# antoine311200/sow

Measured on AMD Instinct MI355X. Metric: SoWLinear fwd+bwd tokens/s, llama_60m rank=50 (56-layer SoWLinear stack), higher is better.
Workload: dtype bf16

## Files before the change

### include/sow_amd.h

```cpp
#ifndef SOW_AMD_H
#define SOW_AMD_H

#include <stddef.h>
#include <stdint.h>

#ifdef __cplusplus
extern "C" {
#endif

#define SOW_DTYPE_F32 0
#define SOW_DTYPE_BF16 1
#define SOW_DTYPE_F16 2

#define SOW_PARAM_F32 0x100

#define SOW_OK 0
#define SOW_ERR_NULL (-1)
#define SOW_ERR_SHAPE (-2)
#define SOW_ERR_DTYPE (-3)
#define SOW_ERR_ALIGN (-4)
#define SOW_ERR_WORKSPACE (-5)
#define SOW_ERR_UNSUPPORTED (-6)

#define SOW_ACC_NONE 0
#define SOW_ACC_LOWRANK 1
#define SOW_ACC_DENSE 2

#define SOW_H_COLS 64

int sow_version(void);
const char* sow_error_string(int code);

int sow_set_switch(const char* name, int value);
int sow_get_switch(const char* name);

size_t sow_workspace_bytes(int64_t T, int d_in, int d_out, int r_live, int r_acc, int acc_kind, int dtype);
size_t sow_forward_workspace_bytes(int64_t T, int d_in, int d_out, int r_live, int r_acc, int acc_kind, int dtype);
size_t sow_h_save_elems(int64_t T, int r_live);

int sow_forward(const void* x, const void* A, const void* B, const void* acc_down, const void* acc_up, const void* bias,
                void* y, void* h_save, int64_t T, int d_in, int d_out, int r_live, int r_acc, int acc_kind, float scale,
                int dtype, void* workspace, size_t workspace_bytes, void* stream);

int sow_backward(const void* dy, const void* x, const void* h_save, const void* A, const void* B, const void* acc_down,
                 const void* acc_up, void* dx, void* dA, void* dB, void* dbias, int64_t T, int d_in, int d_out,
                 int r_live, int r_acc, int acc_kind, float scale, float grad_beta, int dtype, void* workspace,
                 size_t workspace_bytes, void* stream);

#define SOW_BWD_DATA 1
// ... 123 lines not shown
```

### sow_amd/_lib.py

```python
from __future__ import annotations

import ctypes
import os
from ctypes import POINTER, c_char_p, c_double, c_float, c_int, c_int64, c_size_t, c_void_p

_HERE = os.path.dirname(os.path.abspath(__file__))
LIB_PATH = os.environ.get("SOW_AMD_LIB") or os.path.join(_HERE, "lib", "libsow_amd.so")

F32, BF16, F16 = 0, 1, 2
PARAM_F32 = 0x100
ACC_NONE, ACC_LOWRANK, ACC_DENSE = 0, 1, 2
H_COLS = 64
BWD_DATA, BWD_WEIGHTS, BWD_WEIGHTS_PARTIAL, BWD_WEIGHTS_REDUCE = 1, 2, 4, 8
BWD_GROUP_SLABS = 16
ERR_SHAPE = -2
ERR_UNSUPPORTED = -6



class LayerArgs(ctypes.Structure):
    _fields_ = [("x", c_void_p), ("A", c_void_p), ("B", c_void_p), ("acc_down", c_void_p), ("acc_up", c_void_p),
                ("bias", c_void_p), ("y", c_void_p), ("h_save", c_void_p), ("dy", c_void_p), ("dx", c_void_p),
                ("dA", c_void_p), ("dB", c_void_p), ("dbias", c_void_p), ("T", c_int64), ("d_in", ctypes.c_int32),
                ("d_out", ctypes.c_int32), ("r_live", ctypes.c_int32), ("r_acc", ctypes.c_int32), ("acc_kind", ctypes.c_int32),
# ... 15 lines not shown
                ("in_dims", ctypes.c_int32 * TT_MAX_ORDER), ("out_dims", ctypes.c_int32 * TT_MAX_ORDER),
                ("rows", ctypes.c_int32), ("cols", ctypes.c_int32)]


class TtAdamItem(ctypes.Structure):
    _fields_ = [("m", TtDesc), ("v", TtDesc), ("param", c_void_p), ("grad", c_void_p), ("ld_param", c_int64),
                ("ld_grad", c_int64), ("step_size", c_float), ("lr_times_wd", c_float), ("has_state", ctypes.c_int32),
                ("workspace", c_void_p), ("workspace_bytes", c_size_t)]


SIGNATURES = {
    "sow_version": (c_int, []),
    "sow_error_string": (c_char_p, [c_int]),
    "sow_set_switch": (c_int, [c_char_p, c_int]),
    "sow_get_switch": (c_int, [c_char_p]),
    "sow_workspace_bytes": (c_size_t, [c_int64, c_int, c_int, c_int, c_int, c_int, c_int]),
    "sow_forward_workspace_bytes": (c_size_t, [c_int64, c_int, c_int, c_int, c_int, c_int, c_int]),
    "sow_h_save_elems": (c_size_t, [c_int64, c_int]),
    "sow_forward": (c_int, [c_void_p] * 8 + [c_int64, c_int, c_int, c_int, c_int, c_int, c_float, c_int, c_void_p,
                                               c_size_t, c_void_p]),
    "sow_backward": (c_int, [c_void_p] * 11 + [c_int64, c_int, c_int, c_int, c_int, c_int, c_float, c_float, c_int,
                                                 c_void_p, c_size_t, c_void_p]),
    "sow_backward_ex": (c_int, [c_void_p] * 11 + [c_int64, c_int, c_int, c_int, c_int, c_int, c_float, c_float, c_int,
                                    c_void_p, c_size_t, c_int, c_void_p]),
    "sow_forward_group": (c_int, [POINTER(LayerArgs), c_int, c_int, c_void_p]),
    "sow_backward_group": (c_int, [POINTER(LayerArgs), c_int, c_int, c_int, c_void_p]),
    "sow_forward_shared": (c_int, [POINTER(LayerArgs), c_int, c_int, c_void_p]),
    "sow_backward_shared": (c_int, [POINTER(LayerArgs), c_int, c_int, c_int, c_void_p]),
    "sow_backward_group_reduce_desc": (c_int, [POINTER(LayerArgs), c_int, c_int, c_int, c_void_p, POINTER(c_int)]),
    "sow_backward_group_plan": (c_int, [POINTER(LayerArgs), c_int, c_int, c_int, POINTER(c_int)]),
# ... 57 lines not shown
        msg = load().sow_error_string(code).decode()
        raise SowLibraryError(f"libsow_amd {what} failed with code {code}: {msg}")


class switch:

    def __init__(self, **values):
        self.values = values
        self.old = {}

    @staticmethod
    def _forget_sizes():
        from . import ops
        ops._WS_BYTES.clear()
        ops._FWD_WS_BYTES.clear()

    def __enter__(self):
        lib = load()
        for k, v in self.values.items():
            self.old[k] = lib.sow_get_switch(k.encode())
            check(lib.sow_set_switch(k.encode(), int(v)), f"sow_set_switch({k})")
        self._forget_sizes()
        return self

    def __exit__(self, *exc):
        lib = load()
        for k, v in self.old.items():
            lib.sow_set_switch(k.encode(), v)
        self._forget_sizes()
        return False
# ... 1 lines not shown
```

### sow_amd/csrc/api.hip

```cpp
#include "kernels.hpp"
#include <cstring>
#include <vector>
#include <cstdio>
#include <cstdlib>

namespace sow {

template <typename T, typename TO>
__global__ __launch_bounds__(256) void colsum_kernel(const T* M, int64_t ld, int64_t rows, int D, TO* out, float beta) {
  __shared__ float red[4][64];
  const int c = blockIdx.x * 64 + (threadIdx.x & 63), w = threadIdx.x >> 6;
  float s = 0.f;
  if (c < D)
    for (int64_t i = w; i < rows; i += 4) s += to_f32(M[i * ld + c]);
  red[w][threadIdx.x & 63] = s;
  __syncthreads();
  if (w == 0 && c < D) {
    float v = red[0][threadIdx.x] + red[1][threadIdx.x] + red[2][threadIdx.x] + red[3][threadIdx.x];
    if (beta != 0.f) v += beta * to_f32(out[c]);
    out[c] = from_f32<TO>(v);
  }
}
static int launch_colsum(const void* dy, int64_t T, int d_out, void* dbias, float beta, int dtype, int out_dtype,
                         hipStream_t stream) {
// ... 9 lines not shown
  else if (dtype == SOW_F16 && o32)
    hipLaunchKernelGGL((colsum_kernel<f16_t, float>), grid, dim3(256), 0, stream, (const f16_t*)dy, (int64_t)d_out, T, d_out, (float*)dbias, beta);
  else if (dtype == SOW_F16)
    hipLaunchKernelGGL((colsum_kernel<f16_t, f16_t>), grid, dim3(256), 0, stream, (const f16_t*)dy, (int64_t)d_out, T, d_out, (f16_t*)dbias, beta);
  else
    return SOW_ERR_DTYPE;
  SOW_CHECK_LAUNCH();
  return SOW_OK;
}
}

namespace sow {
static const char* const kSwitchNames[SW_COUNT] = {"FORCE_CHAIN_V1", "NO_SHORT_SPLIT", "NO_FUSED_H", "FORCE_GEMM_V1", "TN_NARROW",
                                                   "NO_GEMM3S",      "GEMM3S",         "GEMM3",      "NO_GROUPED",     "NO_PERSIST",     "NO_NT_STORE",    "NT_LOAD",        "NO_PAIR_FLUSH",  "F32_EXACT",
                                                   "NO_PARK16",      "TN_NO_NT_LOAD",  "NO_TN_ROWS",     "GEMM4",          "NO_GEMM4H",      "NO_CHAIN3F",     "NO_TN_F32Q",     "NO_SPLITK",
                                                   "NO_WIDE_CHAIN",  "NO_SHARED_X",    "NO_RAGGED",      "NO_RAGGED_GEMM"};
static std::atomic<int> g_switch[SW_COUNT];
static std::once_flag g_switch_once;
static void switches_from_env() {
  for (int i = 0; i < SW_COUNT; ++i) {
    char name[64];
    snprintf(name, sizeof name, "SOW_AMD_%s", kSwitchNames[i]);
    const char* v = getenv(name);
    const bool tri = i == SW_GEMM3S || i == SW_GEMM3 || i == SW_GEMM4;
    g_switch[i].store(!v ? -1 : (tri ? (v[0] != '0') : 1), std::memory_order_relaxed);
  }
}
int sw(int which) {
  std::call_once(g_switch_once, switches_from_env);
  return g_switch[which].load(std::memory_order_relaxed);
}
}

using namespace sow;

static inline size_t al256(size_t v) { return (v + 255) & ~(size_t)255; }
static inline size_t esize(int dtype) { return dtype == SOW_F32 ? 4 : 2; }
static inline bool ok_dtype(int d) { return d == SOW_F32 || d == SOW_BF16 || d == SOW_F16; }
static inline bool al4p(const void* p) { return (reinterpret_cast<uintptr_t>(p) & 3) == 0; }
static inline bool al16p(const void* p) { return (reinterpret_cast<uintptr_t>(p) & 15) == 0; }
static inline int split_dtype(int d, bool* pf) {
  *pf = (d & SOW_PARAM_F32) != 0;
  const int cd = d & ~SOW_PARAM_F32;
  if (!ok_dtype(cd) || (*pf && cd == SOW_F32)) return -1;
  return cd;
}
static inline bool flagged(int d) { return (d & SOW_PARAM_F32) != 0; }

constexpr int SHORT_NTB = 128;
// ... 46 lines not shown
    const int g4 = sw(SW_GEMM4);
    const int64_t work = (int64_t)ceil_div(M, 256) * ceil_div(N, 256) * gemm4_splits(M, N, K, false, ws, ws_bytes);
    if (!sw_on(SW_FORCE_GEMM_V1) && (g4 > 0 || (g4 < 0 && work >= 120)) &&
        gemm4_supported(A, lda, B, ldb, transB, nullptr, 0, nullptr, 0, C, ldc, bias, M, N, K, dtype))
      return launch_gemm4(A, lda, B, ldb, transB, nullptr, 0, nullptr, 0, 0, C, ldc, bias, M, N, K, alpha, beta, stream, ws,
                          ws_bytes, dtype);
    return launch_gemm(A, lda, false, B, ldb, transB, C, ldc, bias, M, N, K, alpha, beta, dtype, stream);
  }
  if (gemm2_supported(A, lda, B, ldb, transB, nullptr, 0, nullptr, 0, C, ldc, bias, M, N, K, dtype))
    return launch_gemm2(A, lda, B, ldb, transB, nullptr, 0, nullptr, 0, 0, C, ldc, bias, M, N, K, alpha, beta, stream, ws, ws_bytes);
  return launch_gemm(A, lda, false, B, ldb, transB, C, ldc, bias, M, N, K, alpha, beta, dtype, stream);
}

extern "C" {

int sow_version(void) { return 116; }

int sow_set_switch(const char* name, int value) {
  if (!name) return SOW_ERR_NULL;
  (void)sw(0);
  for (int i = 0; i < SW_COUNT; ++i)
    if (!strcmp(name, kSwitchNames[i])) {
      g_switch[i].store(value < 0 ? -1 : (value != 0), std::memory_order_relaxed);
      return SOW_OK;
    }
  return SOW_ERR_UNSUPPORTED;
}

#ifdef SOW_STAMPS
int sow_debug_set_stamps(void* buf) {
  g_chain2_stamps = buf;
  return SOW_OK;
}
#endif

int sow_get_switch(const char* name) {
  if (!name) return SOW_ERR_NULL;
  for (int i = 0; i < SW_COUNT; ++i)
// ... 254 lines not shown
    if (acc_kind == SOW_ACC_LOWRANK) {
      rc = wide_chain(x, y, acc_down, r_acc, acc_up, d_out, nullptr, nullptr, T, d_in, d_out, r_acc, 1.f, 1.f, 0.f, false, dtype,
                      ws, w, workspace_bytes, stream, true);
      if (rc) return rc;
      beta = 1.f;
    } else if (acc_kind == SOW_ACC_DENSE) {
      rc = rag_dense_product(x, d_in, acc_down, d_out, false, y, d_out, T, d_out, d_in, dtype, stream);
      if (rc) return rc;
      beta = 1.f;
    }
    return wide_chain(x, y, A, r_live, B, d_out, h_save, bias, T, d_in, d_out, r_live, 1.f, scale, beta, false, dtype, ws, w,
                      workspace_bytes, stream, true);
  }
  if (acc_kind == SOW_ACC_DENSE) {
    if (r_live <= 64 && h_save) {
      if (gemm4h_supported(x, d_in, acc_down, d_out, false, A, r_live, B, d_out, y, d_out, bias, h_save, T, d_out, d_in, r_live,
                           dtype))
        return launch_gemm4h(x, d_in, acc_down, d_out, false, A, r_live, B, d_out, y, d_out, bias, h_save, T, d_out, d_in,
                             r_live, scale, dtype, stream);
      if (gemm2h_supported(x, d_in, acc_down, d_out, false, A, r_live, B, d_out, y, d_out, bias, h_save, T, d_out, d_in,
                           r_live, dtype))
        return launch_gemm2h(x, d_in, acc_down, d_out, false, A, r_live, B, d_out, y, d_out, bias, h_save, T, d_out, d_in,
                             r_live, scale, stream);
      ChainParams ph{};
      ph.X = x, ph.Y = nullptr, ph.Hsave = h_save, ph.bias = nullptr;
      ph.M = T, ph.ldx = d_in, ph.ldy = d_out, ph.D1 = d_in, ph.D2 = 0;
      ph.F1b = A, ph.ldf1b = r_live, ph.F2b = B, ph.ldf2b = d_out, ph.rb = r_live;
      ph.scale = scale, ph.beta = 0.f;
      set_planes(ph, ws, w, workspace_bytes);
      if (chain2_supported(ph, dtype) &&
          gemm2_supported(x, d_in, acc_down, d_out, false, h_save, 64, B, d_out, y, d_out, bias, T, d_out, d_in, dtype)) {
        rc = SOW_ERR_UNSUPPORTED;
        if (ws && workspace_bytes >= w.total) rc = launch_chain_short(ph, dtype, false, (float*)(ws + w.off_hp), stream);
        if (rc == SOW_ERR_UNSUPPORTED) rc = launch_chain2(ph, false, dtype, stream);
// ... 131 lines not shown
    rc = wide_chain(dy, dx, B, d_out, A, r_live, dh, nullptr, T, d_out, d_in, r_live, scale, 1.f, beta, true, dtype, ws, w,
                    workspace_bytes, stream, true);
    if (rc) return rc;
    do_data = false;
  }
  if (!do_data) {
  } else if (acc_kind == SOW_ACC_DENSE) {
    if (r_live <= 64) {
      ChainParams pd{};
      pd.X = dy, pd.Y = nullptr, pd.Hsave = dh, pd.bias = nullptr;
      pd.M = T, pd.ldx = d_out, pd.ldy = d_in, pd.D1 = d_out, pd.D2 = 0;
      pd.F1b = B, pd.ldf1b = d_out, pd.F2b = A, pd.ldf2b = r_live, pd.rb = r_live;
      pd.scale = scale, pd.beta = 0.f;
      set_planes(pd, ws, w, workspace_bytes);
      void* apad = ws + w.off_apad;
      if (gemm4h_supported(dy, d_out, acc_down, d_out, true, B, d_out, A, r_live, dx, d_in, nullptr, dh, T, d_in, d_out, r_live,
                           dtype)) {
        rc = launch_gemm4h(dy, d_out, acc_down, d_out, true, B, d_out, A, r_live, dx, d_in, nullptr, dh, T, d_in, d_out, r_live,
                           scale, dtype, stream);
        if (rc) return rc;
        data_done = true;
      } else if (gemm2h_supported(dy, d_out, acc_down, d_out, true, B, d_out, A, r_live, dx, d_in, nullptr, dh, T, d_in, d_out,
                           r_live, dtype)) {
        rc = launch_gemm2h(dy, d_out, acc_down, d_out, true, B, d_out, A, r_live, dx, d_in, nullptr, dh, T, d_in, d_out,
                           r_live, scale, stream);
        if (rc) return rc;
        data_done = true;
      } else if (chain2_supported(pd, dtype) &&
          gemm2_supported(dy, d_out, acc_down, d_out, true, dh, 64, apad, 64, dx, d_in, nullptr, T, d_in, d_out, dtype)) {
        const bool pad_fused = (int64_t)ceil_div(T, 64) * 64 >= d_in;
        if (pad_fused) pd.pad_src = A, pd.pad_dst = apad, pd.pad_rows = d_in, pd.pad_r = r_live;
        rc = SOW_ERR_UNSUPPORTED;
        if (short_hp_bytes(T, d_in, d_out, r_live, dtype)) rc = launch_chain_short(pd, dtype, true, (float*)(ws + w.off_hp), stream);
        if (rc == SOW_ERR_UNSUPPORTED) rc = launch_chain2(pd, true, dtype, stream);
// ... 214 lines not shown
  ChainParams batch[C2_MAXG];
  Gemm2hArgs gbatch[4];
  int nb = 0, ng = 0, rc;
  for (int i = 0; i < n; ++i) {
    const sow_layer_args& L = layers[i];
    if ((rc = check_layer(L, false))) return rc;
    if (L.T == 0) continue;
    const WsPlan w{};
    if (group_chain_params(L, false, dtype, w, &batch[nb])) {
      if (++nb == C2_MAXG) {
        if ((rc = launch_chain2_group(batch, nb, false, dtype, stream))) return rc;
        nb = 0;
      }
      continue;
    }
    if (L.acc_kind == SOW_ACC_DENSE && L.r_live <= 64 && L.h_save &&
        gemm4h_supported(L.x, L.d_in, L.acc_down, L.d_out, false, L.A, L.r_live, L.B, L.d_out, L.y, L.d_out, L.bias, L.h_save, L.T,
                         L.d_out, L.d_in, L.r_live, dtype)) {
      if ((rc = launch_gemm4h(L.x, L.d_in, L.acc_down, L.d_out, false, L.A, L.r_live, L.B, L.d_out, L.y, L.d_out, L.bias, L.h_save,
                              L.T, L.d_out, L.d_in, L.r_live, L.scale, dtype, stream)))
        return rc;
      continue;
    }
    if (L.acc_kind == SOW_ACC_DENSE && L.r_live <= 64 && L.h_save && !sw_on(SW_NO_GROUPED) &&
        gemm2h_supported(L.x, L.d_in, L.acc_down, L.d_out, false, L.A, L.r_live, L.B, L.d_out, L.y, L.d_out, L.bias, L.h_save, L.T,
                         L.d_out, L.d_in, L.r_live, dtype)) {
      gbatch[ng] = Gemm2hArgs{L.x, L.acc_down, L.A, L.B, L.y, L.bias, L.h_save, L.T, L.d_in, L.d_out, L.r_live, L.d_out, L.d_out,
                              L.d_out, L.d_in, L.r_live, L.scale};
      if (++ng == 4) {
        if ((rc = launch_gemm2h_group(gbatch, ng, false, stream))) return rc;
        ng = 0;
      }
      continue;
    }
    rc = sow_forward(L.x, L.A, L.B, L.acc_down, L.acc_up, L.bias, L.y, L.h_save, L.T, L.d_in, L.d_out, L.r_live, L.r_acc,
                     L.acc_kind, L.scale, dtype, L.workspace, L.workspace_bytes, stream_);
    if (rc) return rc;
// ... 40 lines not shown
    for (int i = 0; i < n; ++i) {
      const sow_layer_args& L = layers[i];
      if (L.T == 0) {
        if ((rc = single(L, SOW_BWD_DATA | (phases & ~SOW_BWD_DATA)))) return rc;
        continue;
      }
      const WsPlan w = plan(L);
      if (L.workspace_bytes < w.total + 255) return SOW_ERR_WORKSPACE;
      void* dh = ws_base(L.workspace) + w.off_dh;
      if (group_chain_params(L, true, dtype, w, &batch[nb])) {
        if (++nb == C2_MAXG) {
          if ((rc = launch_chain2_group(batch, nb, true, dtype, stream))) return rc;
          nb = 0;
        }
      } else if (L.acc_kind == SOW_ACC_DENSE && L.r_live <= 64 &&
                 gemm4h_supported(L.dy, L.d_out, L.acc_down, L.d_out, true, L.B, L.d_out, L.A, L.r_live, L.dx, L.d_in, nullptr, dh,
                                  L.T, L.d_in, L.d_out, L.r_live, dtype)) {
        if ((rc = launch_gemm4h(L.dy, L.d_out, L.acc_down, L.d_out, true, L.B, L.d_out, L.A, L.r_live, L.dx, L.d_in, nullptr, dh,
                                L.T, L.d_in, L.d_out, L.r_live, L.scale, dtype, stream)))
          return rc;
      } else if (L.acc_kind == SOW_ACC_DENSE && L.r_live <= 64 && !sw_on(SW_NO_GROUPED) &&
                 gemm2h_supported(L.dy, L.d_out, L.acc_down, L.d_out, true, L.B, L.d_out, L.A, L.r_live, L.dx, L.d_in, nullptr, dh,
                                  L.T, L.d_in, L.d_out, L.r_live, dtype)) {
        gbatch[ng] = Gemm2hArgs{L.dy, L.acc_down, L.B, L.A, L.dx, nullptr, dh, L.T, L.d_out, L.d_out, L.d_out, L.r_live, L.d_in,
                                L.d_in, L.d_out, L.r_live, L.scale};
        if (++ng == 4) {
          if ((rc = launch_gemm2h_group(gbatch, ng, true, stream))) return rc;
          ng = 0;
        }
      } else if ((rc = single(L, SOW_BWD_DATA)))
        return rc;
    }
    if (ng && (rc = launch_gemm2h_group(gbatch, ng, true, stream))) return rc;
    if (nb && (rc = launch_chain2_group(batch, nb, true, dtype, stream))) return rc;
  }
// ... 351 lines not shown
```

### sow_amd/csrc/common.hpp

```cpp
#pragma once
#include <hip/hip_runtime.h>
#include <stdint.h>

#include <atomic>
#include <mutex>

#include "../../include/sow_amd.h"

namespace sow {

typedef __bf16 bf16_t;
typedef __attribute__((ext_vector_type(8))) __bf16 bf16x8;
typedef __attribute__((ext_vector_type(4))) __bf16 bf16x4;
typedef __attribute__((ext_vector_type(2))) __bf16 bf16x2;
typedef _Float16 f16_t;
typedef __attribute__((ext_vector_type(8))) _Float16 f16x8;
typedef __attribute__((ext_vector_type(2))) _Float16 f16x2;
typedef __attribute__((ext_vector_type(16))) float f32x16;
typedef __attribute__((ext_vector_type(4))) float f32x4;
typedef __attribute__((ext_vector_type(2))) float f32x2;
typedef __attribute__((ext_vector_type(4))) uint32_t u32x4;
typedef __attribute__((ext_vector_type(2))) uint32_t u32x2;

enum : int { SOW_F32 = 0, SOW_BF16 = 1, SOW_F16 = 2 };
// ... 110 lines not shown
  SW_NT_LOAD,
  SW_NO_PAIR_FLUSH,
  SW_F32_EXACT,
  SW_NO_PARK16,
  SW_TN_NO_NT_LOAD,
  SW_NO_TN_ROWS,
  SW_GEMM4,
  SW_NO_GEMM4H,
  SW_NO_CHAIN3F,
  SW_NO_TN_F32Q,
  SW_NO_SPLITK,
  SW_NO_WIDE_CHAIN,
  SW_NO_SHARED_X,
  SW_NO_RAGGED,
  SW_NO_RAGGED_GEMM,
  SW_COUNT
};
int sw(int which);
inline bool sw_on(int which) { return sw(which) > 0; }

#ifdef SOW_GEMM_NO_NT
#define SOW_GEMM_NT(M) false
#else
#define SOW_GEMM_NT(M) ((M) >= 8192)
#endif

#define SOW_CHECK_LAUNCH()                     \
  do {                                         \
    hipError_t e__ = hipGetLastError();        \
    if (e__ != hipSuccess) return (int)e__;    \
// ... 4 lines not shown
```

### sow_amd/csrc/kernels.hpp

```cpp
#pragma once
#include "common.hpp"

namespace sow {
struct ChainParams {
  const void* X;
  void* Y;
  const void *F1a, *F1b, *F2a, *F2b;
  void* Hsave;
  const void* bias;
  int64_t M, ldx, ldy, ldf1a, ldf1b, ldf2a, ldf2b;
  int D1, D2, ra, rb;
  float scale, beta;
  int fast_factors;
  const void* pad_src;
  void* pad_dst;
  int pad_rows, pad_r;
  int ntb, st_per, sl_per;
  float* Hpartial;
  const void* Hload;
  int nt_store;
  int nt_load;
  int pair_flush;
  void* planes;
  size_t planes_bytes;
// ... 151 lines not shown
                 float alpha, float beta, hipStream_t stream);
bool gemm4_supported(const void* A, int64_t lda, const void* B, int64_t ldb, bool nt, const void* A2, int64_t lda2,
                     const void* B2, int64_t ldb2, const void* C, int64_t ldc, const void* bias, int64_t M, int N, int K,
                     int dtype);
int launch_gemm4(const void* A, int64_t lda, const void* B, int64_t ldb, bool nt, const void* A2, int64_t lda2,
                 const void* B2, int64_t ldb2, int k2, void* C, int64_t ldc, const void* bias, int64_t M, int N, int K,
                 float alpha, float beta, hipStream_t stream, void* ws = nullptr, size_t ws_bytes = 0, int dtype = SOW_BF16);
size_t gemm4_splitk_bytes(int64_t M, int N, int K, bool has_ext);
int gemm4_splits(int64_t M, int N, int K, bool has_ext, const void* ws, size_t ws_bytes);
bool gemm4h_supported(const void* X, int64_t ldx, const void* W, int64_t ldw, bool nt, const void* F, int64_t ldf,
                      const void* G, int64_t ldg, const void* C, int64_t ldc, const void* bias, const void* H, int64_t M,
                      int N, int K, int r, int dtype);
int launch_gemm4h(const void* X, int64_t ldx, const void* W, int64_t ldw, bool nt, const void* F, int64_t ldf,
                  const void* G, int64_t ldg, void* C, int64_t ldc, const void* bias, void* H, int64_t M, int N, int K,
                  int r, float hscale, int dtype, hipStream_t stream);
bool gemm2h_supported(const void* X, int64_t ldx, const void* W, int64_t ldw, bool nt, const void* F, int64_t ldf,
                      const void* G, int64_t ldg, const void* C, int64_t ldc, const void* bias, const void* H, int64_t M,
                      int N, int K, int r, int dtype);
int launch_gemm2h(const void* X, int64_t ldx, const void* W, int64_t ldw, bool nt, const void* F, int64_t ldf,
                  const void* G, int64_t ldg, void* C, int64_t ldc, const void* bias, void* H, int64_t M, int N, int K,
                  int r, float hscale, hipStream_t stream);
struct Gemm2hArgs {
  const void *X, *W, *F, *G;
  void* C;
  const void* bias;
  void* H;
  int64_t M, ldx, ldw, ldf, ldg, ldc;
  int N, K, r;
  float hscale;
};
// ... 53 lines not shown
```

Before: 8.865 million.

## Add gemm5h fused dense plus low-rank GEMM with H output for wide-N backward

Adds a new bf16/f16 kernel for dense-accumulator layers. It fuses the dense GEMM with the low-rank H projection and its correction into one pass. It uses a 128x512 output tile, a three-stage LDS ring filled by direct-to-LDS DMA, and MFMA 16x16x32, with each dispatch path trying it before the existing gemm4h. By default it runs only for the backward data pass, N up to 512 and large token counts (at least 192 row panels). The aim is to read each X row panel once for the whole output width and to overlap loads with MFMA work. The cost is heavy LDS use per block, which may limit occupancy, and more complex edge patching for ragged F and G.

```diff
diff --git a/include/sow_amd.h b/include/sow_amd.h
--- a/include/sow_amd.h
+++ b/include/sow_amd.h
@@ -33,6 +33,8 @@
 
 int sow_set_switch(const char* name, int value);
 int sow_get_switch(const char* name);
+
+int sow_dense_h_kernel(int64_t T, int d_in, int d_out, int r_live, int dtype, int backward);
 
 size_t sow_workspace_bytes(int64_t T, int d_in, int d_out, int r_live, int r_acc, int acc_kind, int dtype);
 size_t sow_forward_workspace_bytes(int64_t T, int d_in, int d_out, int r_live, int r_acc, int acc_kind, int dtype);
diff --git a/sow_amd/_lib.py b/sow_amd/_lib.py
--- a/sow_amd/_lib.py
+++ b/sow_amd/_lib.py
@@ -53,6 +53,7 @@
     "sow_error_string": (c_char_p, [c_int]),
     "sow_set_switch": (c_int, [c_char_p, c_int]),
     "sow_get_switch": (c_int, [c_char_p]),
+    "sow_dense_h_kernel": (c_int, [c_int64, c_int, c_int, c_int, c_int, c_int]),
     "sow_workspace_bytes": (c_size_t, [c_int64, c_int, c_int, c_int, c_int, c_int, c_int]),
     "sow_forward_workspace_bytes": (c_size_t, [c_int64, c_int, c_int, c_int, c_int, c_int, c_int]),
     "sow_h_save_elems": (c_size_t, [c_int64, c_int]),
@@ -140,6 +141,7 @@
         from . import ops
         ops._WS_BYTES.clear()
         ops._FWD_WS_BYTES.clear()
+        ops._GEMM_WS_BYTES.clear()
 
     def __enter__(self):
         lib = load()
diff --git a/sow_amd/csrc/api.hip b/sow_amd/csrc/api.hip
--- a/sow_amd/csrc/api.hip
+++ b/sow_amd/csrc/api.hip
@@ -47,7 +47,7 @@
 static const char* const kSwitchNames[SW_COUNT] = {"FORCE_CHAIN_V1", "NO_SHORT_SPLIT", "NO_FUSED_H", "FORCE_GEMM_V1", "TN_NARROW",
                                                    "NO_GEMM3S",      "GEMM3S",         "GEMM3",      "NO_GROUPED",     "NO_PERSIST",     "NO_NT_STORE",    "NT_LOAD",        "NO_PAIR_FLUSH",  "F32_EXACT",
                                                    "NO_PARK16",      "TN_NO_NT_LOAD",  "NO_TN_ROWS",     "GEMM4",          "NO_GEMM4H",      "NO_CHAIN3F",     "NO_TN_F32Q",     "NO_SPLITK",
-                                                   "NO_WIDE_CHAIN",  "NO_SHARED_X",    "NO_RAGGED",      "NO_RAGGED_GEMM"};
+                                                   "NO_WIDE_CHAIN",  "NO_SHARED_X",    "NO_RAGGED",      "NO_RAGGED_GEMM", "GEMM5H"};
 static std::atomic<int> g_switch[SW_COUNT];
 static std::once_flag g_switch_once;
 static void switches_from_env() {
@@ -56,7 +56,10 @@
     snprintf(name, sizeof name, "SOW_AMD_%s", kSwitchNames[i]);
     const char* v = getenv(name);
     const bool tri = i == SW_GEMM3S || i == SW_GEMM3 || i == SW_GEMM4;
-    g_switch[i].store(!v ? -1 : (tri ? (v[0] != '0') : 1), std::memory_order_relaxed);
+    if (i == SW_GEMM5H)
+      g_switch[i].store(!v ? -1 : (v[0] >= '0' && v[0] <= '2' ? v[0] - '0' : 1), std::memory_order_relaxed);
+    else
+      g_switch[i].store(!v ? -1 : (tri ? (v[0] != '0') : 1), std::memory_order_relaxed);
   }
 }
 int sw(int which) {
@@ -66,6 +69,16 @@
 }
 
 using namespace sow;
+
+static int launch_dense_h(const void* X, int64_t ldx, const void* W, int64_t ldw, bool nt, const void* F, int64_t ldf,
+                          const void* G, int64_t ldg, void* C, int64_t ldc, const void* bias, void* H, int64_t M, int N, int K,
+                          int r, float hscale, int dtype, hipStream_t stream) {
+  if (gemm5h_supported(X, ldx, W, ldw, nt, F, ldf, G, ldg, C, ldc, bias, H, M, N, K, r, dtype))
+    return launch_gemm5h(X, ldx, W, ldw, nt, F, ldf, G, ldg, C, ldc, bias, H, M, N, K, r, hscale, dtype, stream);
+  if (gemm4h_supported(X, ldx, W, ldw, nt, F, ldf, G, ldg, C, ldc, bias, H, M, N, K, r, dtype))
+    return launch_gemm4h(X, ldx, W, ldw, nt, F, ldf, G, ldg, C, ldc, bias, H, M, N, K, r, hscale, dtype, stream);
+  return SOW_ERR_UNSUPPORTED;
+}
 
 static inline size_t al256(size_t v) { return (v + 255) & ~(size_t)255; }
 static inline size_t esize(int dtype) { return dtype == SOW_F32 ? 4 : 2; }
@@ -142,14 +155,24 @@
 
 extern "C" {
 
-int sow_version(void) { return 116; }
+int sow_version(void) { return 117; }
+
+int sow_dense_h_kernel(int64_t T, int d_in, int d_out, int r_live, int dtype, int backward) {
+  const void* a = reinterpret_cast<const void*>(uintptr_t(256));
+  const bool nt = backward != 0;
+  const int N = nt ? d_in : d_out, K = nt ? d_out : d_in;
+  const int64_t ldf = nt ? d_out : r_live, ldg = nt ? r_live : d_out;
+  if (gemm5h_supported(a, K, a, d_out, nt, a, ldf, a, ldg, a, N, nullptr, a, T, N, K, r_live, dtype)) return 5;
+  if (gemm4h_supported(a, K, a, d_out, nt, a, ldf, a, ldg, a, N, nullptr, a, T, N, K, r_live, dtype)) return 4;
+  return 0;
+}
 
 int sow_set_switch(const char* name, int value) {
   if (!name) return SOW_ERR_NULL;
   (void)sw(0);
   for (int i = 0; i < SW_COUNT; ++i)
     if (!strcmp(name, kSwitchNames[i])) {
-      g_switch[i].store(value < 0 ? -1 : (value != 0), std::memory_order_relaxed);
+      g_switch[i].store(value < 0 ? -1 : (i == SW_GEMM5H && value == 2 ? 2 : (value != 0)), std::memory_order_relaxed);
       return SOW_OK;
     }
   return SOW_ERR_UNSUPPORTED;
@@ -434,10 +457,9 @@
   }
   if (acc_kind == SOW_ACC_DENSE) {
     if (r_live <= 64 && h_save) {
-      if (gemm4h_supported(x, d_in, acc_down, d_out, false, A, r_live, B, d_out, y, d_out, bias, h_save, T, d_out, d_in, r_live,
-                           dtype))
-        return launch_gemm4h(x, d_in, acc_down, d_out, false, A, r_live, B, d_out, y, d_out, bias, h_save, T, d_out, d_in,
-                             r_live, scale, dtype, stream);
+      rc = launch_dense_h(x, d_in, acc_down, d_out, false, A, r_live, B, d_out, y, d_out, bias, h_save, T, d_out, d_in, r_live,
+                          scale, dtype, stream);
+      if (rc != SOW_ERR_UNSUPPORTED) return rc;
       if (gemm2h_supported(x, d_in, acc_down, d_out, false, A, r_live, B, d_out, y, d_out, bias, h_save, T, d_out, d_in,
                            r_live, dtype))
         return launch_gemm2h(x, d_in, acc_down, d_out, false, A, r_live, B, d_out, y, d_out, bias, h_save, T, d_out, d_in,
@@ -599,10 +621,9 @@
       pd.scale = scale, pd.beta = 0.f;
       set_planes(pd, ws, w, workspace_bytes);
       void* apad = ws + w.off_apad;
-      if (gemm4h_supported(dy, d_out, acc_down, d_out, true, B, d_out, A, r_live, dx, d_in, nullptr, dh, T, d_in, d_out, r_live,
-                           dtype)) {
-        rc = launch_gemm4h(dy, d_out, acc_down, d_out, true, B, d_out, A, r_live, dx, d_in, nullptr, dh, T, d_in, d_out, r_live,
-                           scale, dtype, stream);
+      rc = launch_dense_h(dy, d_out, acc_down, d_out, true, B, d_out, A, r_live, dx, d_in, nullptr, dh, T, d_in, d_out, r_live,
+                          scale, dtype, stream);
+      if (rc != SOW_ERR_UNSUPPORTED) {
         if (rc) return rc;
         data_done = true;
       } else if (gemm2h_supported(dy, d_out, acc_down, d_out, true, B, d_out, A, r_live, dx, d_in, nullptr, dh, T, d_in, d_out,
@@ -847,13 +868,13 @@
       }
       continue;
     }
-    if (L.acc_kind == SOW_ACC_DENSE && L.r_live <= 64 && L.h_save &&
-        gemm4h_supported(L.x, L.d_in, L.acc_down, L.d_out, false, L.A, L.r_live, L.B, L.d_out, L.y, L.d_out, L.bias, L.h_save, L.T,
-                         L.d_out, L.d_in, L.r_live, dtype)) {
-      if ((rc = launch_gemm4h(L.x, L.d_in, L.acc_down, L.d_out, false, L.A, L.r_live, L.B, L.d_out, L.y, L.d_out, L.bias, L.h_save,
-                              L.T, L.d_out, L.d_in, L.r_live, L.scale, dtype, stream)))
-        return rc;
-      continue;
+    if (L.acc_kind == SOW_ACC_DENSE && L.r_live <= 64 && L.h_save) {
+      rc = launch_dense_h(L.x, L.d_in, L.acc_down, L.d_out, false, L.A, L.r_live, L.B, L.d_out, L.y, L.d_out, L.bias, L.h_save, L.T,
+                          L.d_out, L.d_in, L.r_live, L.scale, dtype, stream);
+      if (rc != SOW_ERR_UNSUPPORTED) {
+        if (rc) return rc;
+        continue;
+      }
     }
     if (L.acc_kind == SOW_ACC_DENSE && L.r_live <= 64 && L.h_save && !sw_on(SW_NO_GROUPED) &&
         gemm2h_supported(L.x, L.d_in, L.acc_down, L.d_out, false, L.A, L.r_live, L.B, L.d_out, L.y, L.d_out, L.bias, L.h_save, L.T,
@@ -924,11 +945,9 @@
           nb = 0;
         }
       } else if (L.acc_kind == SOW_ACC_DENSE && L.r_live <= 64 &&
-                 gemm4h_supported(L.dy, L.d_out, L.acc_down, L.d_out, true, L.B, L.d_out, L.A, L.r_live, L.dx, L.d_in, nullptr, dh,
-                                  L.T, L.d_in, L.d_out, L.r_live, dtype)) {
-        if ((rc = launch_gemm4h(L.dy, L.d_out, L.acc_down, L.d_out, true, L.B, L.d_out, L.A, L.r_live, L.dx, L.d_in, nullptr, dh,
-                                L.T, L.d_in, L.d_out, L.r_live, L.scale, dtype, stream)))
-          return rc;
+                 (rc = launch_dense_h(L.dy, L.d_out, L.acc_down, L.d_out, true, L.B, L.d_out, L.A, L.r_live, L.dx, L.d_in, nullptr,
+                                      dh, L.T, L.d_in, L.d_out, L.r_live, L.scale, dtype, stream)) != SOW_ERR_UNSUPPORTED) {
+        if (rc) return rc;
       } else if (L.acc_kind == SOW_ACC_DENSE && L.r_live <= 64 && !sw_on(SW_NO_GROUPED) &&
                  gemm2h_supported(L.dy, L.d_out, L.acc_down, L.d_out, true, L.B, L.d_out, L.A, L.r_live, L.dx, L.d_in, nullptr, dh,
                                   L.T, L.d_in, L.d_out, L.r_live, dtype)) {
diff --git a/sow_amd/csrc/common.hpp b/sow_amd/csrc/common.hpp
--- a/sow_amd/csrc/common.hpp
+++ b/sow_amd/csrc/common.hpp
@@ -148,6 +148,7 @@
   SW_NO_SHARED_X,
   SW_NO_RAGGED,
   SW_NO_RAGGED_GEMM,
+  SW_GEMM5H,
   SW_COUNT
 };
 int sw(int which);
diff --git a/sow_amd/csrc/gemm5h.hip b/sow_amd/csrc/gemm5h.hip
--- /dev/null
+++ b/sow_amd/csrc/gemm5h.hip
@@ -0,0 +1,418 @@
+#include "kernels.hpp"
+#include "lds_dma.hpp"
+#include <type_traits>
+
+namespace sow {
+
+constexpr int G5_BM = 128, G5_BN = 512, G5_BK = 32;
+constexpr int G5_THREADS = 512;
+constexpr int G5_XOFF = 0, G5_WOFF = 8192, G5_FOFF = G5_WOFF + 32768;
+constexpr int G5_STAGE = G5_FOFF + 4096;
+constexpr int G5_RING = 3 * G5_STAGE;
+constexpr int G5_HIMG = G5_RING;
+constexpr int G5_LDS = G5_RING + 16384;
+constexpr int G5_SCR_LD = 132;
+constexpr int G5_SCR = 16 * G5_SCR_LD * 4;
+static_assert(8 * G5_SCR <= G5_RING, "the epilogue scratch lives in the ring");
+static_assert(G5_STAGE % 256 == 0, "the k-major fragment addresses XOR their low byte");
+
+struct Gemm5Params {
+  const bf16_t* X;
+  const bf16_t* W;
+  const bf16_t* F;
+  const bf16_t* G;
+  bf16_t* C;
+  const bf16_t* bias;
+  bf16_t* Hout;
+  int64_t M, ldx, ldw, ldf, ldg, ldc;
+  int N, K, r;
+  int k2e;
+  float hscale;
+  int nt_store;
+};
+
+template <typename T> __device__ __forceinline__ f32x4 g5_mfma(u32x4 a, u32x4 b, f32x4 c);
+template <> __device__ __forceinline__ f32x4 g5_mfma<bf16_t>(u32x4 a, u32x4 b, f32x4 c) {
+  return __builtin_amdgcn_mfma_f32_16x16x32_bf16(as_bf16x8(a), as_bf16x8(b), c, 0, 0, 0);
+}
+template <> __device__ __forceinline__ f32x4 g5_mfma<f16_t>(u32x4 a, u32x4 b, f32x4 c) {
+  return __builtin_amdgcn_mfma_f32_16x16x32_f16(as_v8<f16_t>(a), as_v8<f16_t>(b), c, 0, 0, 0);
+}
+
+template <int OFF> __device__ __forceinline__ void g5_rd128(u32x4& d, uint32_t a) {
+  asm volatile("ds_read_b128 %0, %1 offset:%2" : "=v"(d) : "v"(a), "n"(OFF) : "memory");
+}
+template <int OFF> __device__ __forceinline__ void g5_rdtr(u32x2& d, uint32_t a) {
+  asm volatile("ds_read_b64_tr_b16 %0, %1 offset:%2" : "=v"(d) : "v"(a), "n"(OFF) : "memory");
+}
+template <bool NT, int CT> __device__ __forceinline__ void g5_rd_tile(u32x4& full, u32x2& lo, u32x2& hi, uint32_t wa, uint32_t fa) {
+  if constexpr (CT < 8) {
+    if constexpr (NT) {
+      g5_rd128<CT * 1024>(full, wa);
+    } else {
+      const uint32_t a = wa ^ (uint32_t)(CT << 5);
+      g5_rdtr<0>(lo, a);
+      g5_rdtr<1024>(hi, a);
+    }
+  } else {
+    if constexpr (NT) {
+      g5_rd128<0>(full, fa);
+    } else {
+      g5_rdtr<0>(lo, fa);
+      g5_rdtr<512>(hi, fa);
+    }
+  }
+}
+
+template <typename T, bool NT> __global__ __launch_bounds__(G5_THREADS, 2) void gemm5h_kernel(const Gemm5Params p) {
+  extern __shared__ __attribute__((aligned(16))) char smem[];
+  const int t = threadIdx.x, lane = t & 63;
+  const int w = __builtin_amdgcn_readfirstlane(t >> 6);
+  const int wr = w >> 2, wc = w & 3;
+  const int r16 = lane & 15, g = lane >> 4;
+  const int lid = xcd_remap(blockIdx.x, gridDim.x);
+  const int64_t m0 = (int64_t)lid * G5_BM;
+  const int K = p.K, N = p.N, r = p.r;
+  const int64_t M = p.M;
+  const int NTA = (K + G5_BK - 1) / G5_BK;
+  const char* zp = zero_page_for(lane);
+  const bool fw = w < 4;
+
+  const int c_row = lane >> 2, c_k = 8 * (lane & 3);
+  const bf16_t* pX;
+  {
+    const int64_t gr = m0 + 16 * w + c_row;
+    pX = p.X + (gr < M ? gr : M - 1) * p.ldx + c_k;
+  }
+  const bf16_t* pW[4];
+  int64_t g_eoff[4];
+  int n_kr[4];
+#pragma unroll
+  for (int ii = 0; ii < 4; ++ii) {
+    if constexpr (NT) {
+      int col = 16 * (4 * w + ii) + c_row;
+      col = col < N ? col : N - 1;
+      pW[ii] = p.W + (int64_t)col * p.ldw + c_k;
+      g_eoff[ii] = (int64_t)col * p.ldg + c_k;
+      n_kr[ii] = 0;
+    } else {
+      const int kr = 16 * (w & 1) + 4 * ii + (lane >> 4);
+      const int f = ((kr & 3) | (((kr >> 3) & 1) << 2)) << 1;
+      int gn = 128 * (w >> 1) + 8 * ((lane & 15) ^ f);
+      gn = gn + 8 <= N ? gn : N - 8;
+      pW[ii] = p.W + (int64_t)kr * p.ldw + gn;
+      g_eoff[ii] = gn;
+      n_kr[ii] = kr;
+    }
+  }
+  const int64_t stepW = NT ? (int64_t)G5_BK : (int64_t)G5_BK * p.ldw;
+  const int f_row = NT ? 16 * w + c_row : 8 * w + (lane >> 3);
+  const int f_q = (lane & 7) ^ ((((lane >> 4) & 1) | ((w & 1) << 1)) << 1);
+  const int64_t f_end = (int64_t)K * p.ldf;
+
+  int ibuf = 0;
+  auto issue = [&](int tl) {
+    char* st = smem + ibuf * G5_STAGE;
+    ibuf = ibuf == 2 ? 0 : ibuf + 1;
+    const int k0 = tl * G5_BK;
+    const bool kin = k0 + c_k < K;
+    dma16(kin ? (const void*)pX : (const void*)zp, st + G5_XOFF + w * 1024);
+    pX += G5_BK;
+#pragma unroll
+    for (int ii = 0; ii < 4; ++ii) {
+      const bool ok = NT ? kin : (k0 + n_kr[ii] < K);
+      dma16(ok ? (const void*)pW[ii] : (const void*)zp, st + G5_WOFF + (4 * w + ii) * 1024);
+      pW[ii] += stepW;
+    }
+    if (fw) {
+      const void* fs;
+      if constexpr (NT) {
+        fs = (f_row < r && kin) ? (const void*)(p.F + (int64_t)f_row * p.ldf + k0 + c_k) : (const void*)zp;
+      } else {
+        const int gk = k0 + f_row;
+        const int64_t eoff = (int64_t)gk * p.ldf + 8 * f_q;
+        fs = (gk < K && 8 * f_q < r && eoff + 8 <= f_end) ? (const void*)(p.F + eoff) : (const void*)zp;
+      }
+      dma16(fs, st + G5_FOFF + w * 1024);
+    }
+  };
+  auto patch_f = [&](int tl, int buf) {
+    if constexpr (!NT) {
+      const int gk = tl * G5_BK + f_row;
+      const int64_t eoff = (int64_t)gk * p.ldf + 8 * f_q;
+      if (fw && gk < K && 8 * f_q < r && eoff + 8 > f_end) {
+        u32x4 v;
+        bf16_t* e = (bf16_t*)&v;
+#pragma unroll
+        for (int j = 0; j < 8; ++j) e[j] = (8 * f_q + j < r) ? p.F[eoff + j] : (bf16_t)0.f;
+        *(u32x4*)(smem + buf * G5_STAGE + G5_FOFF + w * 1024 + lane * 16) = v;
+        asm volatile("s_waitcnt lgkmcnt(0)" ::: "memory");
+      }
+    }
+  };
+  auto issue_g = [&](int ks, int buf) {
+    char* st = smem + buf * G5_STAGE;
+#pragma unroll
+    for (int ii = 0; ii < 4; ++ii) {
+      const void* src;
+      if constexpr (NT) {
+        const int kk = 32 * ks + c_k;
+        const int64_t eoff = g_eoff[ii] + 32 * ks;
+        src = (kk < p.k2e && eoff + 8 <= (int64_t)N * p.ldg) ? (const void*)(p.G + eoff) : (const void*)zp;
+      } else {
+        const int kr = 32 * ks + n_kr[ii];
+        src = kr < r ? (const void*)(p.G + (int64_t)kr * p.ldg + g_eoff[ii]) : (const void*)zp;
+      }
+      dma16(src, st + G5_WOFF + (4 * w + ii) * 1024);
+    }
+  };
+  auto patch_g = [&](int ks, int buf) {
+    if constexpr (NT) {
+#pragma unroll
+      for (int ii = 0; ii < 4; ++ii) {
+        const int kk = 32 * ks + c_k;
+        const int64_t eoff = g_eoff[ii] + 32 * ks;
+        if (kk < p.k2e && eoff + 8 > (int64_t)N * p.ldg) {
+          u32x4 v;
+          bf16_t* e = (bf16_t*)&v;
+#pragma unroll
+          for (int j = 0; j < 8; ++j) e[j] = (kk + j < p.k2e) ? p.G[eoff + j] : (bf16_t)0.f;
+          *(u32x4*)(smem + buf * G5_STAGE + G5_WOFF + (4 * w + ii) * 1024 + lane * 16) = v;
+        }
+      }
+    }
+  };
+
+  const uint32_t base = lds_addr(smem);
+  const int lp = r16 * 4 + g;
+  const uint32_t x_rd = base + (uint32_t)(G5_XOFF + (64 * wr) * 64 + lp * 16);
+  uint32_t w_rd, f_rd;
+  if constexpr (NT) {
+    w_rd = base + (uint32_t)(G5_WOFF + (128 * wc) * 64 + lp * 16);
+    f_rd = base + (uint32_t)(G5_FOFF + (16 * wc) * 64 + lp * 16);
+  } else {
+    const int qq = r16 >> 2, pp = r16 & 3;
+    const int f = (qq | ((g & 1) << 2)) << 1;
+    w_rd = base + (uint32_t)(G5_WOFF + wc * 8192 + (8 * g + qq) * 256 + ((f | (pp >> 1)) << 4) + 8 * (pp & 1));
+    const int ff = (((qq >> 1) & 1) | ((g & 1) << 1)) << 1;
+    f_rd = base + (uint32_t)(G5_FOFF + (8 * g + qq) * 128 + (((wc * 2 + (pp >> 1)) ^ ff) << 4) + 8 * (pp & 1));
+  }
+  const int hsw = (r16 >> 1) & 7;
+  const int hch = (hsw & 4) | (g ^ (hsw & 3));
+  const uint32_t h_rd0 = base + (uint32_t)(G5_HIMG + (64 * wr + r16) * 128 + hch * 16);
+  const uint32_t h_rd1 = base + (uint32_t)(G5_HIMG + (64 * wr + r16) * 128 + (hch ^ 4) * 16);
+
+  f32x4 acc[4][9];
+#pragma unroll
+  for (int a = 0; a < 4; ++a)
+#pragma unroll
+    for (int b = 0; b < 9; ++b) acc[a][b] = (f32x4){0.f, 0.f, 0.f, 0.f};
+
+  using I0 = std::integral_constant<int, 0>;
+  using I1 = std::integral_constant<int, 1>;
+  using I2 = std::integral_constant<int, 2>;
+  using B0 = std::integral_constant<bool, false>;
+  using B1 = std::integral_constant<bool, true>;
+  u32x4 xa[4];
+  u32x4 wf[2][3];
+  u32x2 wl[2][3], wh[2][3];
+  auto rd_group = [&](auto gi_c, auto ext_c, uint32_t wa, uint32_t fa) {
+    constexpr int GI = decltype(gi_c)::value, BUF = GI & 1;
+    constexpr bool EXT = decltype(ext_c)::value;
+    g5_rd_tile<NT, 3 * GI + 0>(wf[BUF][0], wl[BUF][0], wh[BUF][0], wa, fa);
+    g5_rd_tile<NT, 3 * GI + 1>(wf[BUF][1], wl[BUF][1], wh[BUF][1], wa, fa);
+    if constexpr (!(EXT && GI == 2)) g5_rd_tile<NT, 3 * GI + 2>(wf[BUF][2], wl[BUF][2], wh[BUF][2], wa, fa);
+  };
+  auto mma_group = [&](auto gi_c, auto ext_c) {
+    constexpr int GI = decltype(gi_c)::value, BUF = GI & 1;
+    constexpr bool EXT = decltype(ext_c)::value;
+    constexpr int NJ = (EXT && GI == 2) ? 2 : 3;
+#pragma unroll
+    for (int j = 0; j < NJ; ++j) {
+      u32x4 fr;
+      if constexpr (NT) fr = wf[BUF][j];
+      else fr = join2(wl[BUF][j], wh[BUF][j]);
+#pragma unroll
+      for (int mt = 0; mt < 4; ++mt) acc[mt][3 * GI + j] = g5_mfma<T>(fr, xa[mt], acc[mt][3 * GI + j]);
+    }
+  };
+  auto step = [&](auto ext_c, uint32_t xaddr, uint32_t wa, uint32_t fa) {
+    constexpr bool EXT = decltype(ext_c)::value;
+    constexpr int XS = EXT ? 2048 : 1024;
+    g5_rd128<0 * XS>(xa[0], xaddr);
+    g5_rd128<1 * XS>(xa[1], xaddr);
+    g5_rd128<2 * XS>(xa[2], xaddr);
+    g5_rd128<3 * XS>(xa[3], xaddr);
+    rd_group(I0{}, ext_c, wa, fa);
+    asm volatile("s_waitcnt lgkmcnt(0)" ::: "memory");
+    __builtin_amdgcn_sched_barrier(0);
+    rd_group(I1{}, ext_c, wa, fa);
+    __builtin_amdgcn_sched_barrier(0);
+    mma_group(I0{}, ext_c);
+    __builtin_amdgcn_sched_barrier(0);
+    asm volatile("s_waitcnt lgkmcnt(0)" ::: "memory");
+    __builtin_amdgcn_sched_barrier(0);
+    rd_group(I2{}, ext_c, wa, fa);
+    __builtin_amdgcn_sched_barrier(0);
+    mma_group(I1{}, ext_c);
+    __builtin_amdgcn_sched_barrier(0);
+    asm volatile("s_waitcnt lgkmcnt(0)" ::: "memory");
+    __builtin_amdgcn_sched_barrier(0);
+    mma_group(I2{}, ext_c);
+    __builtin_amdgcn_sched_barrier(0);
+  };
+
+  issue(0);
+  issue(1);
+  int cbuf = 0;
+#pragma unroll 1
+  for (int tl = 0; tl < NTA; ++tl) {
+    const int newer = tl + 1 < NTA ? 1 : 0;
+    if (fw) wait_groups<6>(newer);
+    else wait_groups<5>(newer);
+    if (tl == NTA - 1) patch_f(tl, cbuf);
+    __builtin_amdgcn_s_barrier();
+    __builtin_amdgcn_sched_barrier(0);
+    if (tl + 2 < NTA) {
+      issue(tl + 2);
+    } else if (tl == NTA - 1) {
+      issue_g(0, cbuf == 2 ? 0 : cbuf + 1);
+      issue_g(1, cbuf == 0 ? 2 : cbuf - 1);
+    }
+    __builtin_amdgcn_sched_barrier(0);
+    const uint32_t bo = (uint32_t)(cbuf * G5_STAGE);
+    step(B0{}, x_rd + bo, w_rd + bo, f_rd + bo);
+    cbuf = cbuf == 2 ? 0 : cbuf + 1;
+  }
+
+#pragma unroll
+  for (int mt = 0; mt < 4; ++mt) {
+    const int lr = 64 * wr + 16 * mt + r16;
+    const int q = wc * 2 + (g >> 1);
+    f32x4 v = acc[mt][8];
+#pragma unroll
+    for (int j = 0; j < 4; ++j) v[j] = (16 * wc + 4 * g + j < r) ? v[j] * p.hscale : 0.f;
+    *(u32x2*)(smem + G5_HIMG + lr * 128 + ((q ^ ((lr >> 1) & 7)) * 16) + (g & 1) * 8) =
+        (u32x2){pack16x2<T>(v[0], v[1]), pack16x2<T>(v[2], v[3])};
+  }
+  const int gb0 = cbuf, gb1 = cbuf == 2 ? 0 : cbuf + 1;
+  asm volatile("s_waitcnt vmcnt(0)" ::: "memory");
+  __builtin_amdgcn_sched_barrier(0);
+  if constexpr (NT) {
+    if (p.ldg != 64) patch_g(0, gb0), patch_g(1, gb1);
+  }
+  asm volatile("s_waitcnt vmcnt(0) lgkmcnt(0)" ::: "memory");
+  __builtin_amdgcn_s_barrier();
+  __builtin_amdgcn_sched_barrier(0);
+  step(B1{}, h_rd0, w_rd + (uint32_t)(gb0 * G5_STAGE), 0u);
+  step(B1{}, h_rd1, w_rd + (uint32_t)(gb1 * G5_STAGE), 0u);
+  __builtin_amdgcn_s_barrier();
+  __builtin_amdgcn_sched_barrier(0);
+
+  float* sc = (float*)(smem + w * G5_SCR);
+  const bool nts = p.nt_store != 0;
+#pragma unroll
+  for (int mt = 0; mt < 4; ++mt) {
+#pragma unroll
+    for (int ct = 0; ct < 8; ++ct) *(f32x4*)(sc + r16 * G5_SCR_LD + ct * 16 + 4 * g) = acc[mt][ct];
+    __builtin_amdgcn_wave_barrier();
+#pragma unroll
+    for (int pass = 0; pass < 4; ++pass) {
+      const int rr = pass * 4 + (lane >> 4), c = (lane & 15) * 8;
+      const int64_t grow = m0 + 64 * wr + 16 * mt + rr;
+      const int gcol = 128 * wc + c;
+      if (grow < M && gcol < N) {
+        const f32x4 t0 = *(const f32x4*)(sc + rr * G5_SCR_LD + c), t1 = *(const f32x4*)(sc + rr * G5_SCR_LD + c + 4);
+        float v[8] = {t0[0], t0[1], t0[2], t0[3], t1[0], t1[1], t1[2], t1[3]};
+        if (p.bias) {
+          const u32x4 bv = *(const u32x4*)(p.bias + gcol);
+          const T* b = (const T*)&bv;
+#pragma unroll
+          for (int j = 0; j < 8; ++j) v[j] += (float)b[j];
+        }
+        u32x4 pk;
+#pragma unroll
+        for (int j = 0; j < 4; ++j) pk[j] = pack16x2<T>(v[2 * j], v[2 * j + 1]);
+        bf16_t* dst = p.C + grow * p.ldc + gcol;
+        if (nts) asm volatile("global_store_dwordx4 %0, %1, off nt\n\ts_nop 1" ::"v"(dst), "v"(pk) : "memory");
+        else *(u32x4*)dst = pk;
+      }
+    }
+    __builtin_amdgcn_wave_barrier();
+  }
+#pragma unroll
+  for (int it = 0; it < 2; ++it) {
+    const int idx = it * G5_THREADS + t;
+    const int lr = idx >> 3, pc = idx & 7;
+    const int q = pc ^ ((lr >> 1) & 7);
+    const int64_t grow = m0 + lr;
+    if (grow < M) {
+      u32x4 v = *(const u32x4*)(smem + G5_HIMG + lr * 128 + pc * 16);
+      if (q == 7 && r < 64) v[3] = (v[3] & 0xffffu) | (DT<T>::one_bits << 16);
+      *(u32x4*)(p.Hout + grow * 64 + q * 8) = v;
+    }
+  }
+}
+
+static bool g5_al16(const void* q) { return (reinterpret_cast<uintptr_t>(q) & 15) == 0; }
+static bool g5_al4(const void* q) { return (reinterpret_cast<uintptr_t>(q) & 3) == 0; }
+
+constexpr int G5_MIN_PANELS = 192;
+
+bool gemm5h_shape_ok(int64_t M, int N, int K, int r) {
+  return M >= 1 && N >= 8 && N <= G5_BN && N % 8 == 0 && K >= 64 && K % 8 == 0 && r >= 2 && r <= 64 && !(r & 1);
+}
+
+bool gemm5h_supported(const void* X, int64_t ldx, const void* W, int64_t ldw, bool nt, const void* F, int64_t ldf,
+                      const void* G, int64_t ldg, const void* C, int64_t ldc, const void* bias, const void* H, int64_t M,
+                      int N, int K, int r, int dtype) {
+  if ((dtype != SOW_BF16 && dtype != SOW_F16) || !X || !W || !F || !G || !C || !H) return false;
+  const int mode = sw(SW_GEMM5H);
+  if (mode == 0) return false;
+  if (sw_on(SW_NO_FUSED_H) || sw_on(SW_FORCE_GEMM_V1) || sw(SW_GEMM4) == 0 || sw_on(SW_NO_GEMM4H)) return false;
+  if (!gemm5h_shape_ok(M, N, K, r)) return false;
+  if (mode != 2 && (!nt || ceil_div(M, G5_BM) < G5_MIN_PANELS)) return false;
+  if (ceil_div(M, G5_BM) <= 0) return false;
+  if (ldx % 8 || ldw % 8 || ldc % 8) return false;
+  if (!g5_al16(X) || !g5_al16(W) || !g5_al16(C) || !g5_al16(H) || (bias && !g5_al16(bias))) return false;
+  if (nt) {
+    if (ldf % 8 || !g5_al16(F) || !g5_al4(G) || (ldg != r && ldg != 64)) return false;
+  } else {
+    if (ldg % 8 || !g5_al16(G) || !g5_al4(F) || (ldf != r && ldf != 64)) return false;
+  }
+  return true;
+}
+
+int launch_gemm5h(const void* X, int64_t ldx, const void* W, int64_t ldw, bool nt, const void* F, int64_t ldf,
+                  const void* G, int64_t ldg, void* C, int64_t ldc, const void* bias, void* H, int64_t M, int N, int K,
+                  int r, float hscale, int dtype, hipStream_t stream) {
+  if (dtype != SOW_BF16 && dtype != SOW_F16) return SOW_ERR_DTYPE;
+  if (!gemm5h_shape_ok(M, N, K, r) || !H) return SOW_ERR_SHAPE;
+  Gemm5Params p;
+  p.X = (const bf16_t*)X, p.W = (const bf16_t*)W, p.F = (const bf16_t*)F, p.G = (const bf16_t*)G;
+  p.C = (bf16_t*)C, p.bias = (const bf16_t*)bias, p.Hout = (bf16_t*)H;
+  p.M = M, p.ldx = ldx, p.ldw = ldw, p.ldf = ldf, p.ldg = ldg, p.ldc = ldc;
+  p.N = N, p.K = K, p.r = r;
+  p.k2e = nt ? (ldg == 64 ? 64 : r) : 64;
+  p.hscale = hscale;
+  p.nt_store = SOW_GEMM_NT(M) ? 1 : 0;
+  const int64_t panels = (M + G5_BM - 1) / G5_BM;
+  if (panels > 0x7fffffff) return SOW_ERR_SHAPE;
+#define G5_LAUNCH(...)                                                                                                     \
+  do {                                                                                                                     \
+    SOW_SET_MAX_LDS_ONCE(G5_LDS, gemm5h_kernel<__VA_ARGS__>);                                                              \
+    hipLaunchKernelGGL((gemm5h_kernel<__VA_ARGS__>), dim3((unsigned)panels), dim3(G5_THREADS), G5_LDS, stream, p);        \
+  } while (0)
+  if (dtype == SOW_F16) {
+    if (nt) G5_LAUNCH(f16_t, true);
+    else G5_LAUNCH(f16_t, false);
+  } else {
+    if (nt) G5_LAUNCH(bf16_t, true);
+    else G5_LAUNCH(bf16_t, false);
+  }
+#undef G5_LAUNCH
+  SOW_CHECK_LAUNCH();
+  return SOW_OK;
+}
+
+}
diff --git a/sow_amd/csrc/kernels.hpp b/sow_amd/csrc/kernels.hpp
--- a/sow_amd/csrc/kernels.hpp
+++ b/sow_amd/csrc/kernels.hpp
@@ -189,6 +189,13 @@
 int launch_gemm4h(const void* X, int64_t ldx, const void* W, int64_t ldw, bool nt, const void* F, int64_t ldf,
                   const void* G, int64_t ldg, void* C, int64_t ldc, const void* bias, void* H, int64_t M, int N, int K,
                   int r, float hscale, int dtype, hipStream_t stream);
+bool gemm5h_shape_ok(int64_t M, int N, int K, int r);
+bool gemm5h_supported(const void* X, int64_t ldx, const void* W, int64_t ldw, bool nt, const void* F, int64_t ldf,
+                      const void* G, int64_t ldg, const void* C, int64_t ldc, const void* bias, const void* H, int64_t M,
+                      int N, int K, int r, int dtype);
+int launch_gemm5h(const void* X, int64_t ldx, const void* W, int64_t ldw, bool nt, const void* F, int64_t ldf,
+                  const void* G, int64_t ldg, void* C, int64_t ldc, const void* bias, void* H, int64_t M, int N, int K,
+                  int r, float hscale, int dtype, hipStream_t stream);
 bool gemm2h_supported(const void* X, int64_t ldx, const void* W, int64_t ldw, bool nt, const void* F, int64_t ldf,
                       const void* G, int64_t ldg, const void* C, int64_t ldc, const void* bias, const void* H, int64_t M,
                       int N, int K, int r, int dtype);
```

After: 8.833 million. No clear change (-0.4%).
